# liupei101/AdvMIL

Measured on AMD Instinct MI355X. Metric: WSI bags/sec (full G+D step), higher is better.
Workload: dtype bf16x3 (fp32 operands split hi+lo, 3 bf16 MFMAs per product, fp32 accumulate; fp32 storage); 1 GPU; ABMIL+AdvMIL(RLIP prj discriminator), 8192-patch x 1024 fp32 bags (BASELINE.json configs[1] shape; fp32 storage, bf16x3 split arithmetic: >= the bf16 the config names, within 2e-5 of the fp32 reference); gen_updates=1, distinct_resident_bags_per_gpu=64, parallelism=bag-parallel dp1, dropout=shipped rates, launch=hipGraph replay (4 captured bag groups)

## Files before the change

advmil_amd/csrc/gemm_nt_planes.hip:

```cpp
#include "gemm_core.h"


template <int TN, int NBUF, int WR, int BKT, int EPI = 0, int ALO = 1>
__global__ __launch_bounds__(128 * WR, 2) void gemm_nt_planes_kernel(GemmArgs g) {
  constexpr int TM = 2, WC = 2, NW = WR * WC;
  constexpr int BM_ = 64 * WR, BN_ = 64 * TN;
  constexpr int AROWS = (1 + ALO) * BM_;
  constexpr int ROWS_ALL = AROWS + 2 * BN_;
  constexpr int RPP = 512 / BKT, LPR = BKT / 8;
  constexpr int NPIECE = ROWS_ALL / RPP, PPW = NPIECE / NW;
  static_assert(NPIECE % NW == 0, "pieces must divide evenly over the waves");
  constexpr int BUF_HW = ROWS_ALL * BKT;
  constexpr int PATCH_FLOATS = NW * EPI_WAVE_FLOATS(TM, TN);
  constexpr bool EPI_IN_SLOT = PATCH_FLOATS <= BUF_HW / 2;
  static_assert(EPI_IN_SLOT || ALO == 0, "the epilogue area must fit one ring slot");
  constexpr int EST = TM * TN * 4;
  static_assert(EST + PPW <= 63, "counted waits are 6-bit");
  __shared__ __attribute__((aligned(16))) float smem[NBUF * BUF_HW / 2 + (EPI_IN_SLOT ? 0 : PATCH_FLOATS)];
  bf16raw* const lds = reinterpret_cast<bf16raw*>(smem);
  const int wave = __builtin_amdgcn_readfirstlane((int)threadIdx.x >> 6);
  const int wr = wave / WC, wc = wave % WC;
  const int ntile = g.mtiles * g.ntiles, G = (int)gridDim.x;
  auto tile_of = [&](int v, int& mt, int& nt) {
    const int inner = g.ntiles, outer = g.mtiles;
    const int per_group = 8 * inner, full = (outer / 8) * per_group;
    if (v < full) {
      const int r = v % per_group;
      mt = (v / per_group) * 8 + (r & 7);
      nt = r >> 3;
    } else {
      const int rem = outer - (outer / 8) * 8, r = v - full;
      mt = (outer / 8) * 8 + r % rem;
      nt = r / rem;
    }
  };
  int v = (int)blockIdx.x;
  int mt_i, nt_i;
  tile_of(v, mt_i, nt_i);
  uint32_t soff[PPW];
  auto set_src = [&](int mt, int nt, int lane) {
#pragma unroll
    for (int it = 0; it < PPW; ++it) {
      const int prow = (wave + NW * it) * RPP + lane / LPR;
      int r;
      int64_t ld, row0;
      if (prow < BM_) { r = prow; ld = g.lda; row0 = (int64_t)mt * BM_; }
      else if (prow < AROWS) { r = prow - BM_; ld = g.lda; row0 = (int64_t)mt * BM_; }
      else if (prow < AROWS + BN_) { r = prow - AROWS; ld = g.ldb; row0 = (int64_t)nt * BN_; }
      else { r = prow - AROWS - BN_; ld = g.ldb; row0 = (int64_t)nt * BN_; }
      soff[it] = (uint32_t)(((row0 + r) * ld + ps_unit(r, lane % LPR, LPR) * 8) * 2);
    }
  };
  set_src(mt_i, nt_i, (int)threadIdx.x & 63);
  int64_t dA = 0, dB = 0;
  auto dma = [&](int buf, int64_t k0, bool next) {
#pragma unroll
    for (int it = 0; it < PPW; ++it) {
      const int p0 = (wave + NW * it) * RPP;
      const char* base = reinterpret_cast<const char*>(p0 < BM_ ? g.epi.a_hi : (p0 < AROWS ? g.epi.a_lo : (p0 < AROWS + BN_ ? g.epi.b_hi : g.epi.b_lo)));
      base += (k0 + (next ? (p0 < AROWS ? dA : dB) : 0)) * 2;
      __builtin_amdgcn_global_load_lds((const GLB_AS void*)(base + soff[it]), (LDS_AS void*)(lds + buf * BUF_HW + (wave + NW * it) * 512), 16, 0, 0);
    }
  };
  const int64_t K = g.K;
  const int C = (int)(K / BKT);
  dma(0, 0, false);
  if (NBUF == 3) dma(1, BKT, false);
  int cur = 0;
  int young = 0;
  for (; v < ntile; v += G) {
    int lane = (int)threadIdx.x & 63;
    asm volatile("" : "+v"(lane));
    const int i = lane & 31, hi = lane >> 5;
    const bool has_next = v + G < ntile;
    const int64_t m0 = (int64_t)mt_i * BM_, n0 = (int64_t)nt_i * BN_;
    int mt_n = mt_i, nt_n = nt_i;
    if (has_next) tile_of(v + G, mt_n, nt_n);
    dA = (int64_t)(mt_n - mt_i) * BM_ * g.lda;
    dB = (int64_t)(nt_n - nt_i) * BN_ * g.ldb;
    f32x16 acc[TM][TN];
#pragma unroll
    for (int a = 0; a < TM; ++a)
#pragma unroll
      for (int b = 0; b < TN; ++b)
#pragma unroll
        for (int r = 0; r < 16; ++r) acc[a][b][r] = 0.0f;
    for (int c = 0; c < C; ++c) {
      const bool more = c + 1 < C || has_next;
      if constexpr (NBUF == 3) {
        const bool st = young && c < 2;
        if (more) { if (st) wait_vmcnt<PPW + EST>(); else wait_vmcnt<PPW>(); }
        else { if (st) wait_vmcnt<EST>(); else wait_vmcnt<0>(); }
      } else {
        if (young && c == 0) wait_vmcnt<EST>(); else wait_vmcnt<0>();
      }
      __builtin_amdgcn_s_barrier();
      asm volatile("" ::: "memory");
      {
        const int pc = c + NBUF - 1;
        const int pbuf = cur == 0 ? NBUF - 1 : cur - 1;
        if (pc < C) dma(pbuf, (int64_t)pc * BKT, false);
        else if (has_next) dma(pbuf, (int64_t)(pc - C) * BKT, true);
      }
      const bf16raw* cA = lds + cur * BUF_HW;
      const bf16raw* cB = cA + AROWS * BKT;
#pragma unroll
      for (int ks = 0; ks < BKT / 16; ++ks) {
        bf16x8 ah[TM], al[TM], bh[TN], bl[TN];
#pragma unroll
        for (int a = 0; a < TM; ++a) {
          if constexpr (ALO) read_frag_presplit<BM_, BKT>(cA, wr * 32 * TM + a * 32, ks, i, hi, ah[a], al[a]);
          else read_frag_hi<BKT>(cA, wr * 32 * TM + a * 32, ks, i, hi, ah[a]);
        }
#pragma unroll
        for (int b = 0; b < TN; ++b) read_frag_presplit<BN_, BKT>(cB, wc * 32 * TN + b * 32, ks, i, hi, bh[b], bl[b]);
#pragma unroll
        for (int a = 0; a < TM; ++a)
#pragma unroll
          for (int b = 0; b < TN; ++b) {
            if constexpr (ALO) acc[a][b] = __builtin_amdgcn_mfma_f32_32x32x16_bf16(al[a], bh[b], acc[a][b], 0, 0, 0);
            acc[a][b] = __builtin_amdgcn_mfma_f32_32x32x16_bf16(ah[a], bl[b], acc[a][b], 0, 0, 0);
            acc[a][b] = __builtin_amdgcn_mfma_f32_32x32x16_bf16(ah[a], bh[b], acc[a][b], 0, 0, 0);
          }
      }
      cur = cur == NBUF - 1 ? 0 : cur + 1;
    }
    const int last = cur == 0 ? NBUF - 1 : cur - 1;
    young = gemm_epilogue<TM, TN, WR, WC, true, EPI>(g, acc, EPI_IN_SLOT ? smem + last * (BUF_HW / 2) : smem + NBUF * (BUF_HW / 2), wave, lane, wr,
                                                     wc, m0, n0, 0, nt_i);
    mt_i = mt_n; nt_i = nt_n;
    if (has_next) {
      int lane2 = (int)threadIdx.x & 63;
      asm volatile("" : "+v"(lane2));
      set_src(mt_i, nt_i, lane2);
    }
  }
}


int advmil_launch_nt_planes(int tile, bool a_single, dim3 pgrid, hipStream_t stream, const GemmArgs& g) {
  if (a_single) {
    switch (tile) {
      case 85: hipLaunchKernelGGL((gemm_nt_planes_kernel<4, 2, 4, 32, 2, 0>), pgrid, dim3(512), 0, stream, g); break;
      case 86: hipLaunchKernelGGL((gemm_nt_planes_kernel<2, 3, 4, 32, 2, 0>), pgrid, dim3(512), 0, stream, g); break;
      case 83: hipLaunchKernelGGL((gemm_nt_planes_kernel<3, 2, 4, 32, 0, 0>), pgrid, dim3(512), 0, stream, g); break;
      case 82: hipLaunchKernelGGL((gemm_nt_planes_kernel<2, 3, 4, 32, 0, 0>), pgrid, dim3(512), 0, stream, g); break;
      default: return ADVMIL_EINVAL;
    }
    ADVMIL_LAUNCH_CHECK();
    return ADVMIL_OK;
  }
  switch (tile) {
    case 84: hipLaunchKernelGGL((gemm_nt_planes_kernel<4, 2, 4, 32, 1>), pgrid, dim3(512), 0, stream, g); break;
    case 85: hipLaunchKernelGGL((gemm_nt_planes_kernel<4, 2, 4, 32, 2>), pgrid, dim3(512), 0, stream, g); break;
    case 86: hipLaunchKernelGGL((gemm_nt_planes_kernel<2, 3, 4, 32, 2>), pgrid, dim3(512), 0, stream, g); break;
    case 83: hipLaunchKernelGGL((gemm_nt_planes_kernel<3, 2, 4, 32>), pgrid, dim3(512), 0, stream, g); break;
    case 82: hipLaunchKernelGGL((gemm_nt_planes_kernel<2, 3, 4, 32>), pgrid, dim3(512), 0, stream, g); break;
    default: return ADVMIL_EINVAL;
  }
  ADVMIL_LAUNCH_CHECK();
  return ADVMIL_OK;
}
```

Before: 5757 bags/s.

## Add two-phase software-pipelined NT planes GEMM with interleaved DMA and fragment reads

```diff
diff --git a/advmil_amd/csrc/gemm_nt_planes.hip b/advmil_amd/csrc/gemm_nt_planes.hip
--- a/advmil_amd/csrc/gemm_nt_planes.hip
+++ b/advmil_amd/csrc/gemm_nt_planes.hip
@@ -1,7 +1,35 @@
+#include <type_traits>
+
 #include "gemm_core.h"
 
 
-template <int TN, int NBUF, int WR, int BKT, int EPI = 0, int ALO = 1>
+#ifdef NT_STAMP
+#define NT_ST_WG 256
+__device__ unsigned long long g_nt_stamps[NT_ST_WG * 2 * 8];
+extern "C" int advmil_debug_nt_stamps(unsigned long long* dst, int n) { return (int)hipMemcpyFromSymbol(dst, HIP_SYMBOL(g_nt_stamps), (size_t)n * 8); }
+__device__ __forceinline__ unsigned long long nt_now() {
+  unsigned long long t;
+  __builtin_amdgcn_sched_barrier(0);
+  asm volatile("s_memtime %0\n\ts_waitcnt lgkmcnt(0)" : "=s"(t)::"memory");
+  __builtin_amdgcn_sched_barrier(0);
+  return t;
+}
+#define NT_ST_DECL() unsigned long long st_sum[8] = {0, 0, 0, 0, 0, 0, 0, 0}, st_prev = nt_now(); const bool st_on = (wave & 3) == 0
+#define NT_ST(k) do { if (st_on) { const unsigned long long t_ = nt_now(); st_sum[k] += t_ - st_prev; st_prev = t_; } } while (0)
+#define NT_ST_COUNT(k) do { st_sum[k] += 1; } while (0)
+#define NT_ST_FLUSH()                                                                                       \
+  do {                                                                                                      \
+    if (st_on && ((int)threadIdx.x & 63) == 0 && blockIdx.x < NT_ST_WG)                                     \
+      for (int q_ = 0; q_ < 8; ++q_) g_nt_stamps[((int)blockIdx.x * 2 + (wave >> 2)) * 8 + q_] = st_sum[q_]; \
+  } while (0)
+#else
+#define NT_ST_DECL() do { } while (0)
+#define NT_ST(k) do { } while (0)
+#define NT_ST_COUNT(k) do { } while (0)
+#define NT_ST_FLUSH() do { } while (0)
+#endif
+
+template <int TN, int NBUF, int WR, int BKT, int EPI = 0, int ALO = 1, int PH = 0>
 __global__ __launch_bounds__(128 * WR, 2) void gemm_nt_planes_kernel(GemmArgs g) {
   constexpr int TM = 2, WC = 2, NW = WR * WC;
   constexpr int BM_ = 64 * WR, BN_ = 64 * TN;
@@ -53,87 +81,230 @@
   };
   set_src(mt_i, nt_i, (int)threadIdx.x & 63);
   int64_t dA = 0, dB = 0;
-  auto dma = [&](int buf, int64_t k0, bool next) {
-#pragma unroll
-    for (int it = 0; it < PPW; ++it) {
-      const int p0 = (wave + NW * it) * RPP;
-      const char* base = reinterpret_cast<const char*>(p0 < BM_ ? g.epi.a_hi : (p0 < AROWS ? g.epi.a_lo : (p0 < AROWS + BN_ ? g.epi.b_hi : g.epi.b_lo)));
-      base += (k0 + (next ? (p0 < AROWS ? dA : dB) : 0)) * 2;
-      __builtin_amdgcn_global_load_lds((const GLB_AS void*)(base + soff[it]), (LDS_AS void*)(lds + buf * BUF_HW + (wave + NW * it) * 512), 16, 0, 0);
-    }
+  auto dma_piece = [&](int it, int buf, int64_t k0, bool next) {
+    const int p0 = (wave + NW * it) * RPP;
+    const char* base = reinterpret_cast<const char*>(p0 < BM_ ? g.epi.a_hi : (p0 < AROWS ? g.epi.a_lo : (p0 < AROWS + BN_ ? g.epi.b_hi : g.epi.b_lo)));
+    base += (k0 + (next ? (p0 < AROWS ? dA : dB) : 0)) * 2;
+    __builtin_amdgcn_global_load_lds((const GLB_AS void*)(base + soff[it]), (LDS_AS void*)(lds + buf * BUF_HW + (wave + NW * it) * 512), 16, 0, 0);
   };
-  const int64_t K = g.K;
-  const int C = (int)(K / BKT);
-  dma(0, 0, false);
-  if (NBUF == 3) dma(1, BKT, false);
-  int cur = 0;
-  int young = 0;
-  for (; v < ntile; v += G) {
-    int lane = (int)threadIdx.x & 63;
-    asm volatile("" : "+v"(lane));
-    const int i = lane & 31, hi = lane >> 5;
-    const bool has_next = v + G < ntile;
-    const int64_t m0 = (int64_t)mt_i * BM_, n0 = (int64_t)nt_i * BN_;
-    int mt_n = mt_i, nt_n = nt_i;
-    if (has_next) tile_of(v + G, mt_n, nt_n);
-    dA = (int64_t)(mt_n - mt_i) * BM_ * g.lda;
-    dB = (int64_t)(nt_n - nt_i) * BN_ * g.ldb;
-    f32x16 acc[TM][TN];
-#pragma unroll
-    for (int a = 0; a < TM; ++a)
-#pragma unroll
-      for (int b = 0; b < TN; ++b)
-#pragma unroll
-        for (int r = 0; r < 16; ++r) acc[a][b][r] = 0.0f;
-    for (int c = 0; c < C; ++c) {
-      const bool more = c + 1 < C || has_next;
-      if constexpr (NBUF == 3) {
-        const bool st = young && c < 2;
-        if (more) { if (st) wait_vmcnt<PPW + EST>(); else wait_vmcnt<PPW>(); }
-        else { if (st) wait_vmcnt<EST>(); else wait_vmcnt<0>(); }
-      } else {
-        if (young && c == 0) wait_vmcnt<EST>(); else wait_vmcnt<0>();
-      }
-      __builtin_amdgcn_s_barrier();
-      asm volatile("" ::: "memory");
-      {
-        const int pc = c + NBUF - 1;
-        const int pbuf = cur == 0 ? NBUF - 1 : cur - 1;
-        if (pc < C) dma(pbuf, (int64_t)pc * BKT, false);
-        else if (has_next) dma(pbuf, (int64_t)(pc - C) * BKT, true);
-      }
-      const bf16raw* cA = lds + cur * BUF_HW;
-      const bf16raw* cB = cA + AROWS * BKT;
-#pragma unroll
-      for (int ks = 0; ks < BKT / 16; ++ks) {
-        bf16x8 ah[TM], al[TM], bh[TN], bl[TN];
-#pragma unroll
-        for (int a = 0; a < TM; ++a) {
-          if constexpr (ALO) read_frag_presplit<BM_, BKT>(cA, wr * 32 * TM + a * 32, ks, i, hi, ah[a], al[a]);
-          else read_frag_hi<BKT>(cA, wr * 32 * TM + a * 32, ks, i, hi, ah[a]);
-        }
-#pragma unroll
-        for (int b = 0; b < TN; ++b) read_frag_presplit<BN_, BKT>(cB, wc * 32 * TN + b * 32, ks, i, hi, bh[b], bl[b]);
-#pragma unroll
-        for (int a = 0; a < TM; ++a)
-#pragma unroll
-          for (int b = 0; b < TN; ++b) {
-            if constexpr (ALO) acc[a][b] = __builtin_amdgcn_mfma_f32_32x32x16_bf16(al[a], bh[b], acc[a][b], 0, 0, 0);
-            acc[a][b] = __builtin_amdgcn_mfma_f32_32x32x16_bf16(ah[a], bl[b], acc[a][b], 0, 0, 0);
-            acc[a][b] = __builtin_amdgcn_mfma_f32_32x32x16_bf16(ah[a], bh[b], acc[a][b], 0, 0, 0);
+  if constexpr (PH == 0) {
+    const int64_t K = g.K;
+    const int C = (int)(K / BKT);
+    auto dma = [&](int buf, int64_t k0, bool next) {
+#pragma unroll
+      for (int it = 0; it < PPW; ++it) {
+        const int p0 = (wave + NW * it) * RPP;
+        const char* base = reinterpret_cast<const char*>(p0 < BM_ ? g.epi.a_hi : (p0 < AROWS ? g.epi.a_lo : (p0 < AROWS + BN_ ? g.epi.b_hi : g.epi.b_lo)));
+        base += (k0 + (next ? (p0 < AROWS ? dA : dB) : 0)) * 2;
+        __builtin_amdgcn_global_load_lds((const GLB_AS void*)(base + soff[it]), (LDS_AS void*)(lds + buf * BUF_HW + (wave + NW * it) * 512), 16, 0, 0);
+      }
+    };
+    dma(0, 0, false);
+    if (NBUF == 3) dma(1, BKT, false);
+    int cur = 0;
+    int young = 0;
+    NT_ST_DECL();
+    for (; v < ntile; v += G) {
+      int lane = (int)threadIdx.x & 63;
+      asm volatile("" : "+v"(lane));
+      const int i = lane & 31, hi = lane >> 5;
+      const bool has_next = v + G < ntile;
+      const int64_t m0 = (int64_t)mt_i * BM_, n0 = (int64_t)nt_i * BN_;
+      int mt_n = mt_i, nt_n = nt_i;
+      if (has_next) tile_of(v + G, mt_n, nt_n);
+      dA = (int64_t)(mt_n - mt_i) * BM_ * g.lda;
+      dB = (int64_t)(nt_n - nt_i) * BN_ * g.ldb;
+      f32x16 acc[TM][TN];
+#pragma unroll
+      for (int a = 0; a < TM; ++a)
+#pragma unroll
+        for (int b = 0; b < TN; ++b)
+#pragma unroll
+          for (int r = 0; r < 16; ++r) acc[a][b][r] = 0.0f;
+      NT_ST(5);
+      NT_ST_COUNT(7);
+      for (int c = 0; c < C; ++c) {
+        const bool more = c + 1 < C || has_next;
+        if constexpr (NBUF == 3) {
+          const bool st = young && c < 2;
+          if (more) { if (st) wait_vmcnt<PPW + EST>(); else wait_vmcnt<PPW>(); }
+          else { if (st) wait_vmcnt<EST>(); else wait_vmcnt<0>(); }
+        } else {
+          if (young && c == 0) wait_vmcnt<EST>(); else wait_vmcnt<0>();
+        }
+        NT_ST(0);
+        __builtin_amdgcn_s_barrier();
+        asm volatile("" ::: "memory");
+        NT_ST(1);
+        {
+          const int pc = c + NBUF - 1;
+          const int pbuf = cur == 0 ? NBUF - 1 : cur - 1;
+          if (pc < C) dma(pbuf, (int64_t)pc * BKT, false);
+          else if (has_next) dma(pbuf, (int64_t)(pc - C) * BKT, true);
+        }
+        NT_ST(2);
+        const bf16raw* cA = lds + cur * BUF_HW;
+        const bf16raw* cB = cA + AROWS * BKT;
+#pragma unroll
+        for (int ks = 0; ks < BKT / 16; ++ks) {
+          bf16x8 ah[TM], al[TM], bh[TN], bl[TN];
+#pragma unroll
+          for (int a = 0; a < TM; ++a) {
+            if constexpr (ALO) read_frag_presplit<BM_, BKT>(cA, wr * 32 * TM + a * 32, ks, i, hi, ah[a], al[a]);
+            else read_frag_hi<BKT>(cA, wr * 32 * TM + a * 32, ks, i, hi, ah[a]);
           }
-      }
-      cur = cur == NBUF - 1 ? 0 : cur + 1;
-    }
-    const int last = cur == 0 ? NBUF - 1 : cur - 1;
-    young = gemm_epilogue<TM, TN, WR, WC, true, EPI>(g, acc, EPI_IN_SLOT ? smem + last * (BUF_HW / 2) : smem + NBUF * (BUF_HW / 2), wave, lane, wr,
-                                                     wc, m0, n0, 0, nt_i);
-    mt_i = mt_n; nt_i = nt_n;
-    if (has_next) {
-      int lane2 = (int)threadIdx.x & 63;
-      asm volatile("" : "+v"(lane2));
-      set_src(mt_i, nt_i, lane2);
-    }
+#pragma unroll
+          for (int b = 0; b < TN; ++b) read_frag_presplit<BN_, BKT>(cB, wc * 32 * TN + b * 32, ks, i, hi, bh[b], bl[b]);
+          if (ks == 0) NT_ST(3);
+#pragma unroll
+          for (int a = 0; a < TM; ++a)
+#pragma unroll
+            for (int b = 0; b < TN; ++b) {
+              if constexpr (ALO) acc[a][b] = __builtin_amdgcn_mfma_f32_32x32x16_bf16(al[a], bh[b], acc[a][b], 0, 0, 0);
+              acc[a][b] = __builtin_amdgcn_mfma_f32_32x32x16_bf16(ah[a], bl[b], acc[a][b], 0, 0, 0);
+              acc[a][b] = __builtin_amdgcn_mfma_f32_32x32x16_bf16(ah[a], bh[b], acc[a][b], 0, 0, 0);
+            }
+        }
+        NT_ST(4);
+        NT_ST_COUNT(6);
+        cur = cur == NBUF - 1 ? 0 : cur + 1;
+      }
+      const int last = cur == 0 ? NBUF - 1 : cur - 1;
+      young = gemm_epilogue<TM, TN, WR, WC, true, EPI>(g, acc, EPI_IN_SLOT ? smem + last * (BUF_HW / 2) : smem + NBUF * (BUF_HW / 2), wave, lane, wr,
+                                                       wc, m0, n0, 0, nt_i);
+      mt_i = mt_n; nt_i = nt_n;
+      if (has_next) {
+        int lane2 = (int)threadIdx.x & 63;
+        asm volatile("" : "+v"(lane2));
+        set_src(mt_i, nt_i, lane2);
+      }
+    }
+    NT_ST_FLUSH();
+  } else {
+    static_assert(BKT == 32, "two phases = the two k steps of a 32-deep chunk");
+    constexpr int NG = TM * TN;
+    constexpr int NRC = TM + TN;
+    static_assert(2 * PPW <= 63, "counted waits are 6-bit");
+    const int64_t K = g.K;
+    const int C = (int)(K / BKT);
+    const int D = NBUF == 2 ? 2 : (C >= 3 ? 3 : 2);
+    auto slot_add = [&](int sl, int j) { const int t = sl + j; return t >= NBUF ? t - NBUF : t; };
+#pragma unroll
+    for (int it = 0; it < PPW; ++it) dma_piece(it, 0, 0, false);
+#pragma unroll
+    for (int it = 0; it < PPW; ++it) dma_piece(it, 1, BKT, false);
+    if (D == 3) {
+#pragma unroll
+      for (int it = 0; it < PPW; ++it) dma_piece(it, 2, 2 * BKT, false);
+      wait_vmcnt<2 * PPW>();
+    } else {
+      wait_vmcnt<PPW>();
+    }
+    __builtin_amdgcn_s_barrier();
+    asm volatile("" ::: "memory");
+    int cur = 0;
+    int young = 0;
+    bool carry = false;
+    NT_ST_DECL();
+    for (; v < ntile; v += G) {
+      int lane = (int)threadIdx.x & 63;
+      asm volatile("" : "+v"(lane));
+      const int i = lane & 31, hi = lane >> 5;
+      const bool has_next = v + G < ntile;
+      const int64_t m0 = (int64_t)mt_i * BM_, n0 = (int64_t)nt_i * BN_;
+      int mt_n = mt_i, nt_n = nt_i;
+      if (has_next) tile_of(v + G, mt_n, nt_n);
+      dA = (int64_t)(mt_n - mt_i) * BM_ * g.lda;
+      dB = (int64_t)(nt_n - nt_i) * BN_ * g.ldb;
+      f32x16 acc[TM][TN];
+#pragma unroll
+      for (int a = 0; a < TM; ++a)
+#pragma unroll
+        for (int b = 0; b < TN; ++b)
+#pragma unroll
+          for (int r = 0; r < 16; ++r) acc[a][b][r] = 0.0f;
+      bf16x8 fah[2][TM], fal[2][TM], fbh[2][TN], fbl[2][TN];
+      auto read_call = [&](auto S, const bf16raw* cA, int r) {
+        constexpr int ks = decltype(S)::value;
+        if (r < TM) {
+          if constexpr (ALO) read_frag_presplit<BM_, BKT>(cA, wr * 32 * TM + r * 32, ks, i, hi, fah[ks][r], fal[ks][r]);
+          else read_frag_hi<BKT>(cA, wr * 32 * TM + r * 32, ks, i, hi, fah[ks][r]);
+        } else {
+          read_frag_presplit<BN_, BKT>(cA + AROWS * BKT, wc * 32 * TN + (r - TM) * 32, ks, i, hi, fbh[ks][r - TM], fbl[ks][r - TM]);
+        }
+      };
+      auto phase = [&](auto S, const bf16raw* rA, bool do_dma, int dbuf, int64_t dk0, bool dnext) {
+        constexpr int ks = decltype(S)::value;
+#pragma unroll
+        for (int grp = 0; grp < NG; ++grp) {
+          const int a = grp % TM, b = grp / TM;
+          if constexpr (ALO) acc[a][b] = __builtin_amdgcn_mfma_f32_32x32x16_bf16(fal[ks][a], fbh[ks][b], acc[a][b], 0, 0, 0);
+          acc[a][b] = __builtin_amdgcn_mfma_f32_32x32x16_bf16(fah[ks][a], fbl[ks][b], acc[a][b], 0, 0, 0);
+          acc[a][b] = __builtin_amdgcn_mfma_f32_32x32x16_bf16(fah[ks][a], fbh[ks][b], acc[a][b], 0, 0, 0);
+          if (do_dma) {
+#pragma unroll
+            for (int it = 0; it < PPW; ++it)
+              if (it * NG / PPW == grp) dma_piece(it, dbuf, dk0, dnext);
+          }
+#pragma unroll
+          for (int r = 0; r < NRC; ++r)
+            if (r * (NG - 1) / NRC == grp) read_call(std::integral_constant<int, 1 - ks>{}, rA, r);
+          __builtin_amdgcn_sched_barrier(0);
+        }
+      };
+      NT_ST(5);
+      NT_ST_COUNT(7);
+#pragma unroll
+      for (int r = 0; r < NRC; ++r) read_call(std::integral_constant<int, 0>{}, lds + cur * BUF_HW, r);
+      for (int c = 0; c < C; ++c) {
+        const int nxt = cur == NBUF - 1 ? 0 : cur + 1;
+        NT_ST(3);
+        phase(std::integral_constant<int, 0>{}, lds + cur * BUF_HW, carry && c == 0, slot_add(cur, D - 1), (int64_t)(D - 1) * BKT, false);
+        NT_ST(4);
+        asm volatile("s_waitcnt lgkmcnt(0)" ::: "memory");
+        if constexpr (NBUF == 3) {
+          if (D == 3) {
+            const bool more = c + 2 < C || has_next;
+            const bool st = young && c == 0;
+            if (more) { if (st) wait_vmcnt<PPW + EST>(); else wait_vmcnt<PPW>(); }
+            else { if (st) wait_vmcnt<EST>(); else wait_vmcnt<0>(); }
+          } else {
+            wait_vmcnt<0>();
+          }
+        } else {
+          wait_vmcnt<0>();
+        }
+        NT_ST(0);
+        __builtin_amdgcn_s_barrier();
+        asm volatile("" ::: "memory");
+        NT_ST(1);
+        {
+          const int pc = c + D;
+          const bool here = pc < C;
+          const bool there = !here && has_next && c != C - 1;
+          phase(std::integral_constant<int, 1>{}, lds + nxt * BUF_HW, here || there, slot_add(cur, D), (int64_t)(here ? pc : pc - C) * BKT, there);
+        }
+        NT_ST(2);
+        NT_ST_COUNT(6);
+        cur = nxt;
+      }
+      const int last = cur == 0 ? NBUF - 1 : cur - 1;
+      int lane_e = (int)threadIdx.x & 63;
+      asm volatile("" : "+v"(lane_e));
+      young = gemm_epilogue<TM, TN, WR, WC, true, EPI>(g, acc, EPI_IN_SLOT ? smem + last * (BUF_HW / 2) : smem + NBUF * (BUF_HW / 2), wave, lane_e, wr,
+                                                       wc, m0, n0, 0, nt_i);
+      mt_i = mt_n; nt_i = nt_n;
+      if (has_next) {
+        int lane2 = (int)threadIdx.x & 63;
+        asm volatile("" : "+v"(lane2));
+        set_src(mt_i, nt_i, lane2);
+        asm volatile("s_waitcnt lgkmcnt(0)" ::: "memory");
+        __builtin_amdgcn_s_barrier();
+        asm volatile("" ::: "memory");
+        carry = true;
+      }
+    }
+    NT_ST_FLUSH();
   }
 }
 
@@ -151,8 +322,8 @@
     return ADVMIL_OK;
   }
   switch (tile) {
-    case 84: hipLaunchKernelGGL((gemm_nt_planes_kernel<4, 2, 4, 32, 1>), pgrid, dim3(512), 0, stream, g); break;
-    case 85: hipLaunchKernelGGL((gemm_nt_planes_kernel<4, 2, 4, 32, 2>), pgrid, dim3(512), 0, stream, g); break;
+    case 84: hipLaunchKernelGGL((gemm_nt_planes_kernel<4, 2, 4, 32, 1, 1, 1>), pgrid, dim3(512), 0, stream, g); break;
+    case 85: hipLaunchKernelGGL((gemm_nt_planes_kernel<4, 2, 4, 32, 2, 1, 1>), pgrid, dim3(512), 0, stream, g); break;
     case 86: hipLaunchKernelGGL((gemm_nt_planes_kernel<2, 3, 4, 32, 2>), pgrid, dim3(512), 0, stream, g); break;
     case 83: hipLaunchKernelGGL((gemm_nt_planes_kernel<3, 2, 4, 32>), pgrid, dim3(512), 0, stream, g); break;
     case 82: hipLaunchKernelGGL((gemm_nt_planes_kernel<2, 3, 4, 32>), pgrid, dim3(512), 0, stream, g); break;
```

Measured after the change: 5777 bags/s (median of 6 runs). No clear change (+0.3%).
